# rhymes-ai/Aria

Measured on NVIDIA H100. Metric: Aria-25.3B bf16 prefill tokens/sec, higher is better.
Workload: dtype bf16

## Files before the change

aria_b200/csrc/common.cuh:

```cuda
#pragma once
#include <cuda.h>
#include <cuda_runtime.h>
#include <stdint.h>
#include <stdio.h>

#include "../../include/aria_b200.h"

namespace aria {

#define ARIA_CHECK_ARG(cond)                                                             \
  do {                                                                                   \
    if (!(cond)) {                                                                       \
      fprintf(stderr, "aria_b200: bad argument: %s (%s:%d)\n", #cond, __FILE__, __LINE__); \
      return ARIA_ERR_BAD_ARG;                                                           \
    }                                                                                    \
  } while (0)

inline int check_launch(const char* what) {
  cudaError_t e = cudaGetLastError();
  if (e != cudaSuccess) {
    fprintf(stderr, "aria_b200: launch of %s failed: %s\n", what, cudaGetErrorString(e));
    return ARIA_ERR_CUDA;
  }
  return ARIA_OK;
// ... 48 lines not shown
                   CU_TENSOR_MAP_INTERLEAVE_NONE, swizzle, CU_TENSOR_MAP_L2_PROMOTION_L2_256B,
                   CU_TENSOR_MAP_FLOAT_OOB_FILL_NONE);
  if (r == CUDA_ERROR_INVALID_CONTEXT || r == CUDA_ERROR_NOT_INITIALIZED) {
    cudaFree(0);
    r = enc(tm, dtype, rank, const_cast<void*>(ptr), gdim, gstr, bx, es,
            CU_TENSOR_MAP_INTERLEAVE_NONE, swizzle, CU_TENSOR_MAP_L2_PROMOTION_L2_256B,
            CU_TENSOR_MAP_FLOAT_OOB_FILL_NONE);
  }
  if (r != CUDA_SUCCESS) {
    fprintf(stderr, "aria_b200: cuTensorMapEncodeTiled failed (%d): rank %d ptr %p dims %llu,%llu stride %llu box %u,%u\n",
            (int)r, rank, ptr, (unsigned long long)dims[0], (unsigned long long)(rank > 1 ? dims[1] : 0),
            (unsigned long long)(rank > 1 ? strides_bytes[0] : 0), box[0], rank > 1 ? box[1] : 0);
    return ARIA_ERR_CUDA;
  }
  return ARIA_OK;
}

inline int make_tmap_2d(CUtensorMap* tm, const void* ptr, uint64_t inner, uint64_t outer, uint64_t row_stride_bytes,
                        uint32_t box_inner, uint32_t box_outer, CUtensorMapSwizzle swizzle = CU_TENSOR_MAP_SWIZZLE_128B,
                        CUtensorMapDataType dtype = CU_TENSOR_MAP_DATA_TYPE_BFLOAT16) {
  uint64_t dims[2] = {inner, outer};
  uint64_t str[1] = {row_stride_bytes};
  uint32_t box[2] = {box_inner, box_outer};
  return make_tmap_bf16_swz(tm, ptr, 2, dims, str, box, swizzle, dtype);
}

constexpr int kMaxDevices = 64;
inline int current_device() {
  int dev = 0;
  cudaGetDevice(&dev);
  return (dev >= 0 && dev < kMaxDevices) ? dev : 0;
}
inline int sm_count() {
  static int n[kMaxDevices] = {};
  const int dev = current_device();
  if (!n[dev]) {
    int v = 0;
    cudaDeviceGetAttribute(&v, cudaDevAttrMultiProcessorCount, dev);
    n[dev] = v > 0 ? v : 132;
  }
  return n[dev];
}
template <typename Kernel>
inline cudaError_t ensure_dynamic_smem(bool* flags, Kernel kern, int bytes) {
  const int dev = current_device();
  if (flags[dev]) return cudaSuccess;
  cudaError_t e = cudaFuncSetAttribute(kern, cudaFuncAttributeMaxDynamicSharedMemorySize, bytes);
  if (e == cudaSuccess) flags[dev] = true;
  else fprintf(stderr, "aria_b200: cudaFuncSetAttribute(smem=%d) failed: %s\n", bytes, cudaGetErrorString(e));
  return e;
}

template <auto kernel, typename... Args>
inline int launch_persistent(const char* name, int threads, int smem, int64_t max_tiles, cudaStream_t stream,
                             const Args&... args) {
  static bool attr_set[kMaxDevices] = {};
  if (ensure_dynamic_smem(attr_set, kernel, smem) != cudaSuccess) return ARIA_ERR_CUDA;
  int grid = sm_count();
  if (max_tiles < grid) grid = static_cast<int>(max_tiles);
  if (grid < 1) grid = 1;
  kernel<<<grid, threads, smem, stream>>>(args...);
  return check_launch(name);
}

int grouped_gemm(const void* a, const void* b, const float* b_scale, void* out, const int32_t* offsets, int64_t rows,
                 int64_t k, int64_t n, int32_t groups, int32_t epilogue, cudaStream_t stream);

}
```

aria_b200/csrc/gemm.cu:

```cuda
#include <cuda_fp8.h>

#include "gemm_common.cuh"

namespace aria {

constexpr int GEMM_STAGES = 4;
constexpr int FP8_LAND_STAGES = 3;
constexpr int FP8_CONVERT_WARPS = 3;
template <int BN, bool B_FP8 = false>
constexpr int gemm_smem_bytes() {
  return 1024  + GEMM_STAGES * (A_STAGE_BYTES + BN * BK * 2) + BM * acc_ld(BN) * 4 + 256  +
         (B_FP8 ? FP8_LAND_STAGES * BN * BK : 0);
}
static_assert(gemm_smem_bytes<128, true>() <= 232448, "fp8 landing ring must fit the opt-in shared memory of a block");

ARIA_DEVICE void e4m3x16_to_bf16(const uint4 v, uint4& lo, uint4& hi) {
  const uint32_t w[4] = {v.x, v.y, v.z, v.w};
  uint32_t o[8];
#pragma unroll
  for (int i = 0; i < 4; ++i) {
#pragma unroll
    for (int h = 0; h < 2; ++h) {
      const __half2_raw hr = __nv_cvt_fp8x2_to_halfraw2(static_cast<__nv_fp8x2_storage_t>(w[i] >> (16 * h)), __NV_E4M3);
      const float2 f = __half22float2(__half2(hr));
      o[2 * i + h] = pack_bf16(f.x, f.y);
    }
  }
  lo = make_uint4(o[0], o[1], o[2], o[3]);
  hi = make_uint4(o[4], o[5], o[6], o[7]);
}

template <int BN, bool B_MN>
ARIA_DEVICE void wgmma_tile_k16(float (&acc)[BN / 2], uint64_t da, uint64_t db) {
  if constexpr (BN == 128) wgmma_m64n128_ss<0, B_MN ? 1 : 0>(acc, da, db, 1u);
  else wgmma_m64n144_ss<0, B_MN ? 1 : 0>(acc, da, db, 1u);
}

template <int BN, bool B_MN, int EPI, bool B_FP8 = false>
__global__ void __launch_bounds__(GEMM_THREADS, 1)
gemm_kernel(const __grid_constant__ CUtensorMap tmA, const __grid_constant__ CUtensorMap tmB0,
            const __grid_constant__ CUtensorMap tmB1, const __grid_constant__ CUtensorMap tmB2, const GemmParams p) {
  constexpr int B_STAGE_BYTES = BN * BK * 2;
  constexpr int STAGE_BYTES = A_STAGE_BYTES + B_STAGE_BYTES;
  constexpr int STAGES = GEMM_STAGES;
  constexpr int ACC_LD = acc_ld(BN);
  constexpr int OUT_BN = (EPI == ARIA_EPI_SWIGLU) ? BN / 2 : BN;
  static_assert(BN == 128 || BN == 144, "tile widths with a wgmma wrapper");
  static_assert(!B_FP8 || (B_MN && BN == 128 && EPI != ARIA_EPI_HEADS), "fp8 B: grouped [G, K, N] weights, 128-wide tiles");
  constexpr int LAND_BYTES = BN * BK;

  uint8_t* smem = smem_1024();
  float* stg = reinterpret_cast<float*>(smem + STAGES * STAGE_BYTES);
  const BarrierRing<STAGES> bar(stg + BM * ACC_LD);
  const BarrierRing<FP8_LAND_STAGES> land_bar(bar.empty + STAGES);
  uint8_t* land = reinterpret_cast<uint8_t*>(bar.full) + 256;

  const int warp = threadIdx.x >> 5;
  const int lane = threadIdx.x & 31;
  const int wg = threadIdx.x >> 7;

  if (warp == 0 && lane == 0) {
    prefetch_tmap(&tmA);
    prefetch_tmap(&tmB0);
    if (p.n_seg > 1 || EPI == ARIA_EPI_SWIGLU) prefetch_tmap(&tmB1);
    if (p.n_seg > 2) prefetch_tmap(&tmB2);
    bar.init(B_FP8 ? 1 + FP8_CONVERT_WARPS : 1, CONSUMER_WARPS);
    if constexpr (B_FP8) land_bar.init(1, FP8_CONVERT_WARPS);
    fence_mbar_init();
  }
  __syncthreads();

  const int n_out_total = p.N * (EPI == ARIA_EPI_SWIGLU ? 1 : p.n_seg);
  const int n_tiles = (n_out_total + OUT_BN - 1) / OUT_BN;
  const int k_blocks = (p.K + BK - 1) / BK;
  const uint32_t smem_base = smem_u32(smem);
  const uint32_t full0 = smem_u32(bar.full), empty0 = smem_u32(bar.empty);

  if (wg == 0) {
    setmaxnreg_dec<40>();
    if (warp == 0 && elect_one()) {
      TileSched sched;
      sched.init(p, n_tiles);
      RingPos<STAGES> rp;
      RingPos<FP8_LAND_STAGES> lp;
      for (int t = blockIdx.x;; t += gridDim.x) {
        int grp, m_idx, n_idx, row0, rows;
        if (!sched.decode(t, grp, m_idx, n_idx, row0, rows)) break;
        const int a_row = row0 + m_idx * BM;
        const int bgrp = weight_block(p, grp);
        int b_c0 = 0, b_c1 = 0;
        const CUtensorMap* tb0 = &tmB0;
        const CUtensorMap* tb1 = &tmB1;
        if constexpr (B_MN) {
          b_c0 = bgrp * p.K;
        } else if constexpr (EPI == ARIA_EPI_SWIGLU) {
          b_c0 = b_c1 = n_idx * OUT_BN;
        } else {
          const int col = n_idx * BN;
          const int seg = col / p.N;
          tb0 = seg == 0 ? &tmB0 : (seg == 1 ? &tmB1 : &tmB2);
          b_c0 = col - seg * p.N + bgrp * p.b_group_rows;
        }
        for (int kb = 0; kb < k_blocks; ++kb) {
          const uint32_t fb = full0 + rp.stage * 8;
          const uint32_t sa = smem_base + rp.stage * STAGE_BYTES;
          const uint32_t sb = sa + A_STAGE_BYTES;
          mbar_wait_addr(empty0 + rp.stage * 8, rp.phase ^ 1);
          mbar_arrive_expect_tx_addr(fb, B_FP8 ? A_STAGE_BYTES : STAGE_BYTES);
          tma_load_2d_addr(sa, &tmA, fb, kb * BK, a_row);
          if constexpr (B_MN) {
            uint32_t dst = sb, box_bytes = 64 * BK * 2, bar_addr = fb;
            if constexpr (B_FP8) {
              bar_addr = smem_u32(land_bar.full) + lp.stage * 8;
              mbar_wait_addr(smem_u32(land_bar.empty) + lp.stage * 8, lp.phase ^ 1);
              mbar_arrive_expect_tx_addr(bar_addr, LAND_BYTES);
              dst = smem_u32(land) + lp.stage * LAND_BYTES;
              box_bytes = 64 * BK;
            }
            const int krow = b_c0 + kb * BK;
#pragma unroll
            for (int c = 0; c < BN / 64; ++c)
              tma_load_2d_addr(dst + c * box_bytes, &tmB0, bar_addr, tile_b_col<BN, EPI>(c * 64, n_idx, p.N), krow);
            if constexpr (B_FP8) lp.next();
          } else if constexpr (EPI == ARIA_EPI_SWIGLU) {
            tma_load_2d_addr(sb, tb0, fb, kb * BK, b_c0);
            tma_load_2d_addr(sb + (BN / 2) * BK * 2, tb1, fb, kb * BK, b_c1);
          } else {
            tma_load_2d_addr(sb, tb0, fb, kb * BK, b_c0);
          }
          rp.next();
        }
      }
    } else if constexpr (B_FP8) {
      if (warp > 0) {
        const int ct = threadIdx.x - 32;
        TileSched sched;
        sched.init(p, n_tiles);
        RingPos<STAGES> rp;
        RingPos<FP8_LAND_STAGES> lp;
        for (int t = blockIdx.x;; t += gridDim.x) {
          int grp, m_idx, n_idx, row0, rows;
          if (!sched.decode(t, grp, m_idx, n_idx, row0, rows)) break;
          for (int kb = 0; kb < k_blocks; ++kb) {
            mbar_wait_addr(smem_u32(land_bar.full) + lp.stage * 8, lp.phase);
            const uint8_t* src = land + lp.stage * LAND_BYTES;
            uint8_t* dst = smem + rp.stage * STAGE_BYTES + A_STAGE_BYTES;
#pragma unroll 1
            for (int i = ct; i < LAND_BYTES / 16; i += FP8_CONVERT_WARPS * 32) {
              const uint4 v = *reinterpret_cast<const uint4*>(src + i * 16);
              uint4 lo, hi;
              e4m3x16_to_bf16(v, lo, hi);
              const int r = (i >> 2) & 63, j = 2 * (i & 3);
              uint8_t* row = dst + (i >> 8) * (64 * BK * 2) + r * 128;
              *reinterpret_cast<uint4*>(row + ((j ^ (r & 7)) << 4)) = lo;
              *reinterpret_cast<uint4*>(row + (((j + 1) ^ (r & 7)) << 4)) = hi;
            }
            fence_proxy_async_smem();
            __syncwarp();
            if (lane == 0) {
              mbar_arrive(&bar.full[rp.stage]);
              mbar_arrive(&land_bar.empty[lp.stage]);
            }
            rp.next();
            lp.next();
          }
        }
      }
    }
  } else {
    setmaxnreg_inc<232>();
    const int cw = wg - 1;
    constexpr uint32_t b_lbo = B_MN ? 64 * BK * 2 : 16;
    constexpr uint32_t b_sbo = 1024;
    constexpr uint32_t b_kadv = (B_MN ? 16 * 128 : 32) >> 4;
    const uint64_t da0 = make_smem_desc(smem_base + cw * 64 * 128, 16, 1024);
    const uint64_t db0 = make_smem_desc(smem_base + A_STAGE_BYTES, b_lbo, b_sbo);
    const ConsumerThread ct = consumer_thread(cw, lane);
    TileSched sched;
    sched.init(p, n_tiles);
    RingPos<STAGES> rp;
    for (int t = blockIdx.x;; t += gridDim.x) {
      int grp, m_idx, n_idx, row0, rows;
      if (!sched.decode(t, grp, m_idx, n_idx, row0, rows)) break;
      float acc[BN / 2];
#pragma unroll
      for (int i = 0; i < BN / 2; ++i) acc[i] = 0.f;
      float2 bsc[BN / 8];
      if constexpr (B_FP8) load_col_scales<BN, EPI>(p, grp, n_idx, ct.frag_col, bsc);
      int prev = -1;
      for (int kb = 0; kb < k_blocks; ++kb) {
        mbar_wait_addr(full0 + rp.stage * 8, rp.phase);
        const uint64_t da = da0 + rp.stage * (STAGE_BYTES >> 4);
        const uint64_t db = db0 + rp.stage * (STAGE_BYTES >> 4);
        wgmma_fence();
#pragma unroll
        for (int k = 0; k < BK / 16; ++k) wgmma_tile_k16<BN, B_MN>(acc, da + k * 2, db + k * b_kadv);
        wgmma_commit();
        wgmma_wait<1>();
        if (prev >= 0 && lane == 0) mbar_arrive(&bar.empty[prev]);
        prev = static_cast<int>(rp.stage);
        rp.next();
      }
      wgmma_wait<0>();
      fence_regs(acc);
      if (prev >= 0 && lane == 0) mbar_arrive(&bar.empty[prev]);
      stage_and_epilogue<BN, EPI, B_FP8 ? AccScale::COL : AccScale::NONE>(p, stg, ct, acc, bsc, 1.f, 1.f, n_out_total, grp,
                                                                           m_idx, n_idx, row0, rows);
    }
  }
}

constexpr int W8_BK = 128;
static_assert(BM * W8_BK == A_STAGE_BYTES, "W8A8 A stage = bf16 A stage");

template <int EPI>
__global__ void __launch_bounds__(GEMM_THREADS, 1)
gemm_w8a8_kernel(const __grid_constant__ CUtensorMap tmA, const __grid_constant__ CUtensorMap tmB, const GemmParams p,
                 const float* __restrict__ a_scale) {
  constexpr int BN = 128;
  constexpr int STAGE_BYTES = A_STAGE_BYTES + BN * W8_BK;
  constexpr int STAGES = GEMM_STAGES;
  constexpr int ACC_LD = acc_ld(BN);
  constexpr int OUT_BN = (EPI == ARIA_EPI_SWIGLU) ? BN / 2 : BN;
  static_assert(EPI == ARIA_EPI_LINEAR || EPI == ARIA_EPI_SWIGLU, "W8A8: expert GEMM epilogues");

  uint8_t* smem = smem_1024();
  float* stg = reinterpret_cast<float*>(smem + STAGES * STAGE_BYTES);
  const BarrierRing<STAGES> bar(stg + BM * ACC_LD);

  const int warp = threadIdx.x >> 5;
  const int lane = threadIdx.x & 31;
  const int wg = threadIdx.x >> 7;

  if (warp == 0 && lane == 0) {
    prefetch_tmap(&tmA);
    prefetch_tmap(&tmB);
    bar.init(1, CONSUMER_WARPS);
    fence_mbar_init();
  }
  __syncthreads();

  const int n_tiles = (p.N + OUT_BN - 1) / OUT_BN;
  const int k_blocks = p.K / W8_BK;
  const uint32_t smem_base = smem_u32(smem);
  const uint32_t full0 = smem_u32(bar.full), empty0 = smem_u32(bar.empty);

  if (wg == 0) {
    setmaxnreg_dec<40>();
    if (warp == 0 && elect_one()) {
      TileSched sched;
      sched.init(p, n_tiles);
      RingPos<STAGES> rp;
      for (int t = blockIdx.x;; t += gridDim.x) {
        int grp, m_idx, n_idx, row0, rows;
        if (!sched.decode(t, grp, m_idx, n_idx, row0, rows)) break;
        const int a_row = row0 + m_idx * BM;
        int b_r0, b_r1;
        if constexpr (EPI == ARIA_EPI_SWIGLU) {
          b_r0 = weight_block(p, grp) * 2 * p.N + n_idx * OUT_BN;
          b_r1 = b_r0 + p.N;
        } else {
          b_r0 = weight_block(p, grp) * p.N + n_idx * BN;
// ... 68 lines not shown
  p.out_group_base = static_cast<const uint64_t*>(d->out_group_base);
  p.out_group_row0 = d->out_group_row0;
  p.group_mod = d->group_mod;
  p.b_group_rows = d->b_layout == ARIA_B_GNK ? static_cast<int>(d->n) : 0;
  p.n_seg = swiglu ? 1 : d->n_seg;
  p.act = d->act;
  for (int i = 0; i < 3; ++i) {
    p.bias[i] = static_cast<const __nv_bfloat16*>(d->bias[i]);
    p.out[i] = static_cast<__nv_bfloat16*>(d->out[i]);
  }
  p.residual = static_cast<const __nv_bfloat16*>(d->residual);
  p.ldr = d->ldr;
  p.ldo = d->ldo;
  p.head_dim = d->head_dim;
  p.head_ld = d->head_ld;
  p.rows_per_batch = d->rows_per_batch > 0 ? d->rows_per_batch : static_cast<int>(d->m);
  p.pos0 = d->pos0;
  p.stride_b = d->stride_b;
  p.stride_h = d->stride_h;
  p.rope_mask = d->rope_mask;
  p.rope_cos = static_cast<const __nv_bfloat16*>(d->rope_cos);
  p.rope_sin = static_cast<const __nv_bfloat16*>(d->rope_sin);
  p.position_ids = d->position_ids;
  p.b_scale = b_scale;
  return p;
}

static aria_gemm_desc_t grouped_desc(const void* a, const void* b, void* out, const int32_t* offsets, int64_t rows, int64_t k,
                                     int64_t n, int32_t groups, int32_t epilogue) {
  aria_gemm_desc_t d{};
  d.a = a;
  d.lda = k;
  d.m = rows;
  d.n = n;
  d.k = k;
  d.b[0] = b;
  d.n_seg = 1;
  d.b_layout = ARIA_B_GKN;
  d.num_groups = groups;
  d.group_offsets = offsets;
  d.epilogue = epilogue;
  d.out[0] = out;
  d.ldo = n;
  return d;
}

static int64_t max_tiles(const aria_gemm_desc_t* d, int BN, int64_t groups) {
  const bool swiglu = d->epilogue == ARIA_EPI_SWIGLU;
  const int out_bn = swiglu ? BN / 2 : BN;
  const int64_t n_out_total = d->n * (swiglu ? 1 : d->n_seg);
  return (n_out_total + out_bn - 1) / out_bn * ((d->m + BM - 1) / BM + groups);
}

static int gemm_run(const aria_gemm_desc_t* d, const float* b_scale, cudaStream_t stream) {
  ARIA_CHECK_ARG(d != nullptr);
  ARIA_CHECK_ARG(d->a && d->b[0] && d->out[0]);
  ARIA_CHECK_ARG(d->m >= 0 && d->n > 0 && d->k > 0);
  ARIA_CHECK_ARG(d->n % 8 == 0 && d->k % 8 == 0 && d->lda % 8 == 0);
  ARIA_CHECK_ARG(d->n_seg >= 1 && d->n_seg <= 3);
  ARIA_CHECK_ARG(d->num_groups >= 1 && (d->group_mod >= 0 || d->num_groups % (-d->group_mod) == 0));
  ARIA_CHECK_ARG((reinterpret_cast<uintptr_t>(d->a) & 15) == 0 && (reinterpret_cast<uintptr_t>(d->out[0]) & 15) == 0);
  if (d->m == 0) return ARIA_OK;
  const bool b_mn = d->b_layout == ARIA_B_GKN;
  const bool b_gnk = d->b_layout == ARIA_B_GNK;
  const bool swiglu = d->epilogue == ARIA_EPI_SWIGLU;
  if (b_mn) {
    ARIA_CHECK_ARG(d->n_seg == 1);
    ARIA_CHECK_ARG(d->k % BK == 0 || (d->num_groups == 1 && d->group_mod == 0));
    ARIA_CHECK_ARG(d->n % 64 == 0);
    ARIA_CHECK_ARG(d->epilogue != ARIA_EPI_HEADS);
  } else {
    ARIA_CHECK_ARG(d->num_groups == 1 || d->n_seg == 1);
    if (swiglu) ARIA_CHECK_ARG(d->n_seg == 2 && d->b[1]);
    if (b_gnk) ARIA_CHECK_ARG(d->n_seg == 1 && !swiglu && d->epilogue == ARIA_EPI_LINEAR && d->n % 128 == 0);
    else ARIA_CHECK_ARG(d->num_groups == 1);
  }
  if (d->num_groups > 1) ARIA_CHECK_ARG(d->group_offsets != nullptr);
  if (d->group_counts) ARIA_CHECK_ARG(d->group_offsets != nullptr);
  if (d->out_group_base) ARIA_CHECK_ARG(d->out_group_row0 != nullptr && d->epilogue == ARIA_EPI_LINEAR && d->group_offsets != nullptr);
  ARIA_CHECK_ARG(d->a_rows == 0 || d->a_rows >= d->m);

  int BN = 128;
  if (d->epilogue == ARIA_EPI_HEADS) {
    ARIA_CHECK_ARG(d->head_dim > 0 && d->head_dim % 8 == 0 && d->head_ld >= d->head_dim && d->n % d->head_dim == 0);
    if (d->rope_mask) ARIA_CHECK_ARG(d->head_dim == 128 && d->rope_cos && d->rope_sin);
    if (d->n % 128 != 0) {
      ARIA_CHECK_ARG(!d->rope_mask && d->n % 144 == 0);
      BN = 144;
    }
    for (int s = 0; s < d->n_seg; ++s) ARIA_CHECK_ARG(d->out[s] && d->b[s]);
  } else {
    if (swiglu) ARIA_CHECK_ARG(d->n % 64 == 0);
    if (d->n_seg > 1 && !swiglu) ARIA_CHECK_ARG(d->n % BN == 0);
  }

  CUtensorMap tmA, tmB[3];
  int rc = make_tmap_2d(&tmA, d->a, d->k, d->a_rows > 0 ? d->a_rows : d->m, d->lda * 2, BK, BM);
  if (rc) return rc;
  if (b_mn) {
    const uint64_t ncols = swiglu ? 2 * d->n : d->n;
    const uint64_t n_weights = d->group_mod > 0 ? d->group_mod : (d->group_mod < 0 ? d->num_groups / (-d->group_mod) : d->num_groups);
    rc = b_scale ? make_tmap_2d(&tmB[0], d->b[0], ncols, n_weights * d->k, ncols, 64, BK, CU_TENSOR_MAP_SWIZZLE_NONE,
                                CU_TENSOR_MAP_DATA_TYPE_UINT8)
                 : make_tmap_2d(&tmB[0], d->b[0], ncols, n_weights * d->k, ncols * 2, 64, BK);
    if (rc) return rc;
    tmB[1] = tmB[0];
    tmB[2] = tmB[0];
  } else {
    const int nb = swiglu ? 2 : d->n_seg;
    const uint32_t box_rows = swiglu ? BN / 2 : BN;
    for (int s = 0; s < 3; ++s) {
      const void* ptr = s < nb ? d->b[s] : d->b[0];
      const uint64_t b_rows = b_gnk ? static_cast<uint64_t>(d->group_mod > 0 ? d->group_mod : (d->group_mod < 0 ? d->num_groups / (-d->group_mod) : d->num_groups)) * d->n : d->n;
      rc = make_tmap_2d(&tmB[s], ptr, d->k, b_rows, d->k * 2, BK, box_rows);
      if (rc) return rc;
    }
  }

  const GemmParams p = gemm_params(d, b_scale);
  const int64_t tiles = max_tiles(d, BN, d->num_groups > 1 ? d->num_groups : 0);
#define ARIA_LAUNCH(BN_, MN_, EPI_, ...)                                                                                     \
  return launch_persistent<gemm_kernel<BN_, MN_, EPI_, ##__VA_ARGS__>>("gemm_kernel", GEMM_THREADS,                          \
                                                                       gemm_smem_bytes<BN_, ##__VA_ARGS__>(), tiles, stream, \
                                                                       tmA, tmB[0], tmB[1], tmB[2], p)
  if (b_scale) {
    if (swiglu) ARIA_LAUNCH(128, true, ARIA_EPI_SWIGLU, true);
    ARIA_LAUNCH(128, true, ARIA_EPI_LINEAR, true);
  }
  if (d->epilogue == ARIA_EPI_HEADS) {
    if (BN == 128) ARIA_LAUNCH(128, false, ARIA_EPI_HEADS);
    ARIA_LAUNCH(144, false, ARIA_EPI_HEADS);
  }
  if (swiglu) {
    if (b_mn) ARIA_LAUNCH(128, true, ARIA_EPI_SWIGLU);
    ARIA_LAUNCH(128, false, ARIA_EPI_SWIGLU);
  }
  if (b_mn) ARIA_LAUNCH(128, true, ARIA_EPI_LINEAR);
  ARIA_LAUNCH(128, false, ARIA_EPI_LINEAR);
#undef ARIA_LAUNCH
}

extern "C" int aria_gemm(const aria_gemm_desc_t* d, aria_stream_t stream) {
  return gemm_run(d, nullptr, reinterpret_cast<cudaStream_t>(stream));
}

int aria::grouped_gemm(const void* a, const void* b, const float* b_scale, void* out, const int32_t* offsets, int64_t rows,
                       int64_t k, int64_t n, int32_t groups, int32_t epilogue, cudaStream_t stream) {
  const aria_gemm_desc_t d = grouped_desc(a, b, out, offsets, rows, k, n, groups, epilogue);
  return gemm_run(&d, b_scale, stream);
}

extern "C" int aria_grouped_gemm(const void* a, const void* b, void* out, const int32_t* group_offsets, int64_t rows,
                                 int64_t k, int64_t n, int32_t num_groups, aria_stream_t stream) {
  return grouped_gemm(a, b, nullptr, out, group_offsets, rows, k, n, num_groups, ARIA_EPI_LINEAR,
                      reinterpret_cast<cudaStream_t>(stream));
}

extern "C" int aria_grouped_gemm_fp8(const void* a, const void* b_fp8, const float* b_scale, void* out,
                                     const int32_t* group_offsets, int64_t rows, int64_t k, int64_t n, int32_t num_groups,
                                     int32_t epilogue, aria_stream_t stream) {
  ARIA_CHECK_ARG(a && b_fp8 && b_scale && out && group_offsets);
  ARIA_CHECK_ARG(rows >= 0 && k > 0 && n > 0 && k % BK == 0 && n % 64 == 0 && num_groups >= 1);
  ARIA_CHECK_ARG(epilogue == ARIA_EPI_LINEAR || epilogue == ARIA_EPI_SWIGLU);
  ARIA_CHECK_ARG((reinterpret_cast<uintptr_t>(a) & 15) == 0 && (reinterpret_cast<uintptr_t>(b_fp8) & 15) == 0 &&
                 (reinterpret_cast<uintptr_t>(b_scale) & 15) == 0 && (reinterpret_cast<uintptr_t>(out) & 15) == 0);
  return grouped_gemm(a, b_fp8, b_scale, out, group_offsets, rows, k, n, num_groups, epilogue,
                      reinterpret_cast<cudaStream_t>(stream));
}

extern "C" int aria_grouped_gemm_w8a8(const void* a_fp8, const float* a_scale, const void* b_fp8_nk, const float* b_scale,
                                      void* out, const int32_t* group_offsets, int64_t rows, int64_t k, int64_t n,
                                      int32_t num_groups, int32_t epilogue, aria_stream_t stream_) {
  ARIA_CHECK_ARG(a_fp8 && a_scale && b_fp8_nk && b_scale && out && group_offsets);
  ARIA_CHECK_ARG(rows >= 0 && rows < (int64_t(1) << 31) && k > 0 && n > 0 && k % W8_BK == 0 && n % 64 == 0 && num_groups >= 1);
  ARIA_CHECK_ARG(k <= (1 << 30) && n <= (1 << 29) && static_cast<int64_t>(num_groups) * n * 2 < (int64_t(1) << 31));
  ARIA_CHECK_ARG(epilogue == ARIA_EPI_LINEAR || epilogue == ARIA_EPI_SWIGLU);
  ARIA_CHECK_ARG((reinterpret_cast<uintptr_t>(a_fp8) & 15) == 0 && (reinterpret_cast<uintptr_t>(b_fp8_nk) & 15) == 0 &&
                 (reinterpret_cast<uintptr_t>(b_scale) & 15) == 0 && (reinterpret_cast<uintptr_t>(out) & 15) == 0 &&
                 (reinterpret_cast<uintptr_t>(a_scale) & 3) == 0);
  if (rows == 0) return ARIA_OK;
  const bool swiglu = epilogue == ARIA_EPI_SWIGLU;
  const aria_gemm_desc_t d = grouped_desc(a_fp8, b_fp8_nk, out, group_offsets, rows, k, n, num_groups, epilogue);
  const GemmParams p = gemm_params(&d, b_scale);

  CUtensorMap tmA, tmB;
  int rc = make_tmap_2d(&tmA, a_fp8, k, rows, k, W8_BK, BM, CU_TENSOR_MAP_SWIZZLE_128B, CU_TENSOR_MAP_DATA_TYPE_UINT8);
  if (rc) return rc;
  rc = make_tmap_2d(&tmB, b_fp8_nk, k, num_groups * (swiglu ? 2 * n : n), k, W8_BK, 64, CU_TENSOR_MAP_SWIZZLE_128B,
                    CU_TENSOR_MAP_DATA_TYPE_UINT8);
  if (rc) return rc;

  const int64_t tiles = max_tiles(&d, 128, num_groups);
  constexpr int SMEM = gemm_smem_bytes<128>();
  cudaStream_t stream = reinterpret_cast<cudaStream_t>(stream_);
  if (swiglu)
    return launch_persistent<gemm_w8a8_kernel<ARIA_EPI_SWIGLU>>("gemm_w8a8_kernel", GEMM_THREADS, SMEM, tiles, stream, tmA,
                                                                 tmB, p, a_scale);
  return launch_persistent<gemm_w8a8_kernel<ARIA_EPI_LINEAR>>("gemm_w8a8_kernel", GEMM_THREADS, SMEM, tiles, stream, tmA, tmB,
                                                              p, a_scale);
}

extern "C" int aria_abi_version(void) { return 3; }
extern "C" const char* aria_build_arch(void) { return "sm_90a"; }
```

aria_b200/csrc/gemm_common.cuh:

```cuda
#pragma once
#include "common.cuh"
#include "ptx.cuh"

namespace aria {

constexpr int BM = 128;
constexpr int BK = 64;
constexpr int A_STAGE_BYTES = BM * BK * 2;
constexpr int GEMM_THREADS = 384;
constexpr int CONSUMER_WARPS = 8;
constexpr int acc_ld(int BN) { return BN + 4; }

struct GemmParams {
  int M, N, K;
  int num_groups;
  const int32_t* group_offsets;
  const int32_t* group_counts;
  const uint64_t* out_group_base;
  const int32_t* out_group_row0;
  int b_group_rows;
  int group_mod;
  int n_seg;
  int act;
  const __nv_bfloat16* bias[3];
  const __nv_bfloat16* residual;
  int64_t ldr;
  __nv_bfloat16* out[3];
  int64_t ldo;
  int head_dim, head_ld, rows_per_batch, pos0;
  int64_t stride_b, stride_h;
  int rope_mask;
  const __nv_bfloat16* rope_cos;
  const __nv_bfloat16* rope_sin;
  const int32_t* position_ids;
  const float* b_scale;
};

ARIA_DEVICE int weight_block(const GemmParams& p, int grp) {
  return p.group_mod > 0 ? grp % p.group_mod : (p.group_mod < 0 ? grp / (-p.group_mod) : grp);
}

ARIA_DEVICE uint8_t* smem_1024() {
  extern __shared__ uint8_t smem_raw[];
  return reinterpret_cast<uint8_t*>((reinterpret_cast<uintptr_t>(smem_raw) + 1023) & ~uintptr_t(1023));
}

template <int STAGES>
struct BarrierRing {
  uint64_t* full;
  uint64_t* empty;
  ARIA_DEVICE explicit BarrierRing(void* at) : full(static_cast<uint64_t*>(at)), empty(full + STAGES) {}
  ARIA_DEVICE void init(uint32_t full_arrivals, uint32_t empty_arrivals) const {
    for (int i = 0; i < STAGES; ++i) {
      mbar_init(&full[i], full_arrivals);
      mbar_init(&empty[i], empty_arrivals);
    }
  }
};

template <int STAGES>
struct RingPos {
  uint32_t stage = 0, phase = 0;
  ARIA_DEVICE void next() {
    const bool wrap = ++stage == STAGES;
    stage = wrap ? 0 : stage;
    phase ^= wrap;
  }
};

template <int BN, int EPI>
ARIA_DEVICE int tile_b_col(int x, int n_idx, int N) {
  constexpr int OUT_BN = BN / 2;
  if constexpr (EPI == ARIA_EPI_SWIGLU) return x < OUT_BN ? n_idx * OUT_BN + x : N + n_idx * OUT_BN + x - OUT_BN;
  else return n_idx * BN + x;
}

struct ConsumerThread {
  int cw, frag_row, frag_col, epi_row, half;
};
ARIA_DEVICE ConsumerThread consumer_thread(int cw, int lane) {
  const int tid = threadIdx.x & 127;
  return {cw, cw * 64 + (tid >> 5) * 16 + (lane >> 2), 2 * (lane & 3), cw * 64 + (tid & 63), tid >> 6};
}

template <int BN, int EPI>
ARIA_DEVICE void load_col_scales(const GemmParams& p, int grp, int n_idx, int frag_col, float2 (&bsc)[BN / 8]) {
  const int ncols = EPI == ARIA_EPI_SWIGLU ? 2 * p.N : p.N;
  const float* srow = p.b_scale + static_cast<int64_t>(weight_block(p, grp)) * ncols;
// ... 328 lines not shown
```

aria_b200/csrc/gemm_wgrad.cu:

```cuda
#include "gemm_common.cuh"

namespace aria {

struct WgradParams {
  int Md, Nd, G;
  int n_src;
  const int32_t* offs;
  __nv_bfloat16* out;
};

constexpr int WG_BN = 128;
constexpr int WG_STAGES = 6;
constexpr int WG_STAGE_BYTES = 64 * BM * 2 + 64 * WG_BN * 2;

__global__ void __launch_bounds__(GEMM_THREADS, 1)
wgrad_kernel(const __grid_constant__ CUtensorMap tmA, const __grid_constant__ CUtensorMap tmB, const WgradParams p) {
  uint8_t* smem = smem_1024();
  const BarrierRing<WG_STAGES> bar(smem + WG_STAGES * WG_STAGE_BYTES);
  const int warp = threadIdx.x >> 5, lane = threadIdx.x & 31, wg = threadIdx.x >> 7;

  if (warp == 0 && lane == 0) {
    prefetch_tmap(&tmA);
    prefetch_tmap(&tmB);
    bar.init(1, CONSUMER_WARPS);
// ... 73 lines not shown
            else named_bar_sync(2, 128);
          }
          wgmma_fence();
          for (int k = 0; k < kmax; ++k) wgmma_m64n128_ss<1, 1>(acc, da + k * (2048 >> 4), db + k * (2048 >> 4), 1u);
          wgmma_commit();
          wgmma_wait<1>();
          if (prev >= 0 && lane == 0) mbar_arrive(&bar.empty[prev]);
          prev = static_cast<int>(rp.stage);
          rp.next();
        }
      }
      wgmma_wait<0>();
      fence_regs(acc);
      if (prev >= 0 && lane == 0) mbar_arrive(&bar.empty[prev]);
#pragma unroll
      for (int h = 0; h < 2; ++h) {
        const int m = mi * BM + ct.frag_row + 8 * h;
        if (m >= p.Md) continue;
        __nv_bfloat16* orow = p.out + (static_cast<int64_t>(g) * p.Md + m) * p.Nd + ni * WG_BN;
#pragma unroll
        for (int j = 0; j < WG_BN / 8; ++j) {
          if (ni * WG_BN + 8 * j + 8 <= p.Nd)
            *reinterpret_cast<uint32_t*>(orow + 8 * j + ct.frag_col) = pack_bf16(acc[4 * j + 2 * h], acc[4 * j + 2 * h + 1]);
        }
      }
    }
  }
}

}

using namespace aria;

extern "C" int aria_grouped_wgrad(const void* a, int64_t lda, const void* b, int64_t ldb, void* out, const int32_t* group_offsets,
                                  int64_t rows, int64_t md, int64_t nd, int32_t num_groups, int32_t num_sources,
                                  aria_stream_t stream_) {
  cudaStream_t stream = reinterpret_cast<cudaStream_t>(stream_);
  ARIA_CHECK_ARG(a && b && out && group_offsets && rows >= 0 && md > 0 && nd > 0 && num_groups >= 1 && num_sources >= 1);
  ARIA_CHECK_ARG(md % 8 == 0 && nd % 8 == 0 && lda % 8 == 0 && ldb % 8 == 0 && lda >= md && ldb >= nd);
  CUtensorMap tmA, tmB;
  int rc = make_tmap_2d(&tmA, a, md, rows > 0 ? rows : 1, lda * 2, 64, 64);
  if (rc) return rc;
  rc = make_tmap_2d(&tmB, b, nd, rows > 0 ? rows : 1, ldb * 2, 64, 64);
  if (rc) return rc;
  WgradParams p{};
  p.Md = static_cast<int>(md);
  p.Nd = static_cast<int>(nd);
  p.G = num_groups;
  p.n_src = num_sources;
  p.offs = group_offsets;
  p.out = static_cast<__nv_bfloat16*>(out);
  constexpr int SMEM = WG_STAGES * WG_STAGE_BYTES + 1024 + 256;
  const int64_t tiles = static_cast<int64_t>(num_groups) * ((md + BM - 1) / BM) * ((nd + WG_BN - 1) / WG_BN);
  return launch_persistent<wgrad_kernel>("wgrad_kernel", GEMM_THREADS, SMEM, tiles, stream, tmA, tmB, p);
}
```

aria_b200/csrc/ptx.cuh:

```cuda
#pragma once
#include <cuda.h>
#include <cuda_bf16.h>
#include <cuda_runtime.h>
#include <stdint.h>

namespace aria {

#define ARIA_DEVICE __device__ __forceinline__

ARIA_DEVICE uint32_t smem_u32(const void* p) { return static_cast<uint32_t>(__cvta_generic_to_shared(p)); }

ARIA_DEVICE uint32_t elect_one() {
  uint32_t pred = 0;
  asm volatile(
      "{\n\t.reg .pred P;\n\t"
      "elect.sync _|P, 0xffffffff;\n\t"
      "selp.b32 %0, 1, 0, P;\n\t}\n"
      : "=r"(pred));
  return pred;
}

ARIA_DEVICE void mbar_init(uint64_t* bar, uint32_t count) {
  asm volatile("mbarrier.init.shared::cta.b64 [%0], %1;" ::"r"(smem_u32(bar)), "r"(count));
}
ARIA_DEVICE void fence_mbar_init() { asm volatile("fence.mbarrier_init.release.cluster;" ::: "memory"); }
ARIA_DEVICE void fence_proxy_async_smem() { asm volatile("fence.proxy.async.shared::cta;" ::: "memory"); }

ARIA_DEVICE void mbar_arrive_expect_tx(uint64_t* bar, uint32_t bytes) {
  asm volatile("mbarrier.arrive.expect_tx.shared::cta.b64 _, [%0], %1;" ::"r"(smem_u32(bar)), "r"(bytes)
               : "memory");
}
ARIA_DEVICE void mbar_arrive(uint64_t* bar) {
  asm volatile("mbarrier.arrive.shared::cta.b64 _, [%0];" ::"r"(smem_u32(bar)) : "memory");
}
ARIA_DEVICE bool mbar_try_wait(uint64_t* bar, uint32_t parity) {
  uint32_t ok;
  asm volatile(
      "{\n\t.reg .pred P;\n\t"
      "mbarrier.try_wait.parity.shared::cta.b64 P, [%1], %2;\n\t"
      "selp.b32 %0, 1, 0, P;\n\t}\n"
      : "=r"(ok) : "r"(smem_u32(bar)), "r"(parity) : "memory");
  return ok != 0;
}
ARIA_DEVICE void mbar_wait_addr(uint32_t addr, uint32_t parity) {
  uint32_t ok = 0;
  long long t0 = 0;
  for (uint32_t spin = 0;; ++spin) {
    asm volatile(
        "{\n\t.reg .pred P;\n\t"
        "mbarrier.try_wait.parity.shared::cta.b64 P, [%1], %2;\n\t"
        "selp.b32 %0, 1, 0, P;\n\t}\n"
        : "=r"(ok) : "r"(addr), "r"(parity) : "memory");
    if (ok) return;
    if ((spin & 0xFFF) == 0xFFF) {
      const long long now = clock64();
      if (t0 == 0) t0 = now;
      if (now - t0 > 4000000000ll) __trap();
    }
  }
}
ARIA_DEVICE void mbar_wait(uint64_t* bar, uint32_t parity) { mbar_wait_addr(smem_u32(bar), parity); }
ARIA_DEVICE void mbar_arrive_expect_tx_addr(uint32_t bar_addr, uint32_t bytes) {
  asm volatile("mbarrier.arrive.expect_tx.shared::cta.b64 _, [%0], %1;" ::"r"(bar_addr), "r"(bytes) : "memory");
}

ARIA_DEVICE void tma_load_2d_addr(uint32_t dst, const CUtensorMap* m, uint32_t bar_addr, int c0, int c1) {
  asm volatile(
      "cp.async.bulk.tensor.2d.shared::cluster.global.mbarrier::complete_tx::bytes [%0], [%1, {%3, %4}], [%2];"
      ::"r"(dst), "l"(reinterpret_cast<uint64_t>(m)), "r"(bar_addr), "r"(c0), "r"(c1)
      : "memory");
}
ARIA_DEVICE void prefetch_tmap(const CUtensorMap* m) {
  asm volatile("prefetch.tensormap [%0];" ::"l"(reinterpret_cast<uint64_t>(m)) : "memory");
}
ARIA_DEVICE void tma_load_2d(void* dst, const CUtensorMap* m, uint64_t* bar, int c0, int c1) {
  asm volatile(
      "cp.async.bulk.tensor.2d.shared::cluster.global.mbarrier::complete_tx::bytes [%0], [%1, {%3, %4}], [%2];"
      ::"r"(smem_u32(dst)), "l"(reinterpret_cast<uint64_t>(m)), "r"(smem_u32(bar)), "r"(c0), "r"(c1)
      : "memory");
}
ARIA_DEVICE void tma_load_3d(void* dst, const CUtensorMap* m, uint64_t* bar, int c0, int c1, int c2) {
  asm volatile(
      "cp.async.bulk.tensor.3d.shared::cluster.global.mbarrier::complete_tx::bytes [%0], [%1, {%3, %4, %5}], [%2];"
      ::"r"(smem_u32(dst)), "l"(reinterpret_cast<uint64_t>(m)), "r"(smem_u32(bar)), "r"(c0), "r"(c1), "r"(c2)
      : "memory");
}
ARIA_DEVICE void tma_load_4d(void* dst, const CUtensorMap* m, uint64_t* bar, int c0, int c1, int c2, int c3) {
  asm volatile(
      "cp.async.bulk.tensor.4d.shared::cluster.global.mbarrier::complete_tx::bytes [%0], [%1, {%3, %4, %5, %6}], [%2];"
      ::"r"(smem_u32(dst)), "l"(reinterpret_cast<uint64_t>(m)), "r"(smem_u32(bar)), "r"(c0), "r"(c1), "r"(c2),
      "r"(c3)
      : "memory");
}

ARIA_DEVICE uint64_t make_smem_desc(uint32_t smem_addr, uint32_t lbo_bytes, uint32_t sbo_bytes) {
  uint64_t d = 0;
  d |= static_cast<uint64_t>((smem_addr & 0x3FFFF) >> 4);
  d |= static_cast<uint64_t>((lbo_bytes >> 4) & 0x3FFF) << 16;
  d |= static_cast<uint64_t>((sbo_bytes >> 4) & 0x3FFF) << 32;
  d |= 1ull << 62;
  return d;
}
ARIA_DEVICE uint64_t make_smem_desc_sw32(uint32_t smem_addr, uint32_t sbo_bytes) {
  uint64_t d = 0;
  d |= static_cast<uint64_t>((smem_addr & 0x3FFFF) >> 4);
  d |= static_cast<uint64_t>(1) << 16;
  d |= static_cast<uint64_t>((sbo_bytes >> 4) & 0x3FFF) << 32;
  d |= 3ull << 62;
  return d;
}
ARIA_DEVICE void wgmma_fence() { asm volatile("wgmma.fence.sync.aligned;" ::: "memory"); }
ARIA_DEVICE void wgmma_commit() { asm volatile("wgmma.commit_group.sync.aligned;" ::: "memory"); }
template <int N> ARIA_DEVICE void wgmma_wait() { asm volatile("wgmma.wait_group.sync.aligned %0;" ::"n"(N) : "memory"); }
template <int R> ARIA_DEVICE void fence_regs(float (&d)[R]) {
#pragma unroll
  for (int i = 0; i < R; ++i) asm volatile("" : "+f"(d[i])::"memory");
}
ARIA_DEVICE void named_bar_sync(uint32_t id, uint32_t threads) { asm volatile("bar.sync %0, %1;" ::"r"(id), "r"(threads) : "memory"); }
ARIA_DEVICE void named_bar_arrive(uint32_t id, uint32_t threads) { asm volatile("bar.arrive %0, %1;" ::"r"(id), "r"(threads) : "memory"); }

template <int TA, int TB>
ARIA_DEVICE void wgmma_m64n128_ss(float (&d)[64], uint64_t da, uint64_t db, uint32_t scale_d) {
// ... 89 lines not shown
```

Measured before the change: 16630.

## Pair CTAs in 2-CTA clusters that multicast shared B tiles for dense GEMMs

Dense bf16 GEMMs with long K and at least two M tiles now launch as 2-CTA clusters. The two CTAs take adjacent M tiles of the same N tile, and each loads half of the B tile and multicasts it to both. Empty-slot releases are sent to both CTAs' barriers so a stage is reused only after both consumers finish. This halves B traffic from global/L2 per pair, at the cost of cluster scheduling limits, cross-CTA lockstep and an extra clamp for odd M-tile counts.

```diff
diff --git a/aria_b200/csrc/common.cuh b/aria_b200/csrc/common.cuh
--- a/aria_b200/csrc/common.cuh
+++ b/aria_b200/csrc/common.cuh
@@ -124,14 +124,49 @@
 }
 
 template <auto kernel, typename... Args>
-inline int launch_persistent(const char* name, int threads, int smem, int64_t max_tiles, cudaStream_t stream,
+inline int launch_persistent(const char* name, int threads, int smem, int64_t max_tiles, int cluster, cudaStream_t stream,
                              const Args&... args) {
   static bool attr_set[kMaxDevices] = {};
+  static int max_clusters[kMaxDevices] = {};
   if (ensure_dynamic_smem(attr_set, kernel, smem) != cudaSuccess) return ARIA_ERR_CUDA;
-  int grid = sm_count();
-  if (max_tiles < grid) grid = static_cast<int>(max_tiles);
-  if (grid < 1) grid = 1;
-  kernel<<<grid, threads, smem, stream>>>(args...);
+  if (cluster <= 1) {
+    int grid = sm_count();
+    if (max_tiles < grid) grid = static_cast<int>(max_tiles);
+    if (grid < 1) grid = 1;
+    kernel<<<grid, threads, smem, stream>>>(args...);
+    return check_launch(name);
+  }
+  cudaLaunchConfig_t cfg{};
+  cudaLaunchAttribute attr{};
+  attr.id = cudaLaunchAttributeClusterDimension;
+  attr.val.clusterDim.x = cluster;
+  attr.val.clusterDim.y = 1;
+  attr.val.clusterDim.z = 1;
+  cfg.blockDim = dim3(threads);
+  cfg.dynamicSmemBytes = smem;
+  cfg.stream = stream;
+  cfg.attrs = &attr;
+  cfg.numAttrs = 1;
+  const int dev = current_device();
+  if (!max_clusters[dev]) {
+    cfg.gridDim = dim3(sm_count() / cluster * cluster);
+    int n = 0;
+    const cudaError_t e = cudaOccupancyMaxActiveClusters(&n, kernel, &cfg);
+    if (e != cudaSuccess || n < 1) {
+      fprintf(stderr, "aria_b200: no cluster of %d x %s fits (%s)\n", cluster, name, cudaGetErrorString(e));
+      return ARIA_ERR_CUDA;
+    }
+    max_clusters[dev] = n;
+  }
+  int64_t clusters = max_clusters[dev];
+  if (max_tiles < clusters) clusters = max_tiles;
+  if (clusters < 1) clusters = 1;
+  cfg.gridDim = dim3(static_cast<unsigned>(clusters * cluster));
+  const cudaError_t e = cudaLaunchKernelEx(&cfg, kernel, args...);
+  if (e != cudaSuccess) {
+    fprintf(stderr, "aria_b200: launch of %s failed: %s\n", name, cudaGetErrorString(e));
+    return ARIA_ERR_CUDA;
+  }
   return check_launch(name);
 }
 
diff --git a/aria_b200/csrc/gemm.cu b/aria_b200/csrc/gemm.cu
--- a/aria_b200/csrc/gemm.cu
+++ b/aria_b200/csrc/gemm.cu
@@ -58,35 +58,41 @@
   const int warp = threadIdx.x >> 5;
   const int lane = threadIdx.x & 31;
   const int wg = threadIdx.x >> 7;
+  const bool pair = !B_MN && p.cta_pair;
+  const int n_cta = pair ? 2 : 1;
+  const int rank = pair ? static_cast<int>(cluster_ctarank()) : 0;
 
   if (warp == 0 && lane == 0) {
     prefetch_tmap(&tmA);
     prefetch_tmap(&tmB0);
     if (p.n_seg > 1 || EPI == ARIA_EPI_SWIGLU) prefetch_tmap(&tmB1);
     if (p.n_seg > 2) prefetch_tmap(&tmB2);
-    bar.init(B_FP8 ? 1 + FP8_CONVERT_WARPS : 1, CONSUMER_WARPS);
+    bar.init(B_FP8 ? 1 + FP8_CONVERT_WARPS : 1, CONSUMER_WARPS * n_cta);
     if constexpr (B_FP8) land_bar.init(1, FP8_CONVERT_WARPS);
     fence_mbar_init();
   }
-  __syncthreads();
+  if (pair) cluster_sync();
+  else __syncthreads();
 
   const int n_out_total = p.N * (EPI == ARIA_EPI_SWIGLU ? 1 : p.n_seg);
   const int n_tiles = (n_out_total + OUT_BN - 1) / OUT_BN;
   const int k_blocks = (p.K + BK - 1) / BK;
   const uint32_t smem_base = smem_u32(smem);
   const uint32_t full0 = smem_u32(bar.full), empty0 = smem_u32(bar.empty);
+  const int t0 = blockIdx.x / n_cta, t_step = gridDim.x / n_cta;
 
   if (wg == 0) {
     setmaxnreg_dec<40>();
     if (warp == 0 && elect_one()) {
       TileSched sched;
-      sched.init(p, n_tiles);
+      sched.init(p, n_tiles, BM * n_cta);
       RingPos<STAGES> rp;
       RingPos<FP8_LAND_STAGES> lp;
-      for (int t = blockIdx.x;; t += gridDim.x) {
+      for (int t = t0;; t += t_step) {
         int grp, m_idx, n_idx, row0, rows;
         if (!sched.decode(t, grp, m_idx, n_idx, row0, rows)) break;
-        const int a_row = row0 + m_idx * BM;
+        m_idx = m_idx * n_cta + rank;
+        const int a_row = row0 + min(m_idx, (rows - 1) / BM) * BM;
         const int bgrp = weight_block(p, grp);
         int b_c0 = 0, b_c1 = 0;
         const CUtensorMap* tb0 = &tmB0;
@@ -122,11 +128,17 @@
             for (int c = 0; c < BN / 64; ++c)
               tma_load_2d_addr(dst + c * box_bytes, &tmB0, bar_addr, tile_b_col<BN, EPI>(c * 64, n_idx, p.N), krow);
             if constexpr (B_FP8) lp.next();
-          } else if constexpr (EPI == ARIA_EPI_SWIGLU) {
-            tma_load_2d_addr(sb, tb0, fb, kb * BK, b_c0);
-            tma_load_2d_addr(sb + (BN / 2) * BK * 2, tb1, fb, kb * BK, b_c1);
           } else {
-            tma_load_2d_addr(sb, tb0, fb, kb * BK, b_c0);
+#pragma unroll
+            for (int h = 0; h < 2; ++h) {
+              if (pair && h != rank) continue;
+              const uint32_t dst = sb + h * (BN / 2) * BK * 2;
+              const CUtensorMap* tb = EPI == ARIA_EPI_SWIGLU && h ? tb1 : tb0;
+              int b_row = EPI == ARIA_EPI_SWIGLU ? (h ? b_c1 : b_c0) : b_c0 + h * (BN / 2);
+              if (b_row - bgrp * p.b_group_rows >= p.N) b_row = b_c0;
+              if (pair) tma_load_2d_multicast_addr(dst, tb, fb, kb * BK, b_row, 0x3);
+              else tma_load_2d_addr(dst, tb, fb, kb * BK, b_row);
+            }
           }
           rp.next();
         }
@@ -176,12 +188,21 @@
     const uint64_t da0 = make_smem_desc(smem_base + cw * 64 * 128, 16, 1024);
     const uint64_t db0 = make_smem_desc(smem_base + A_STAGE_BYTES, b_lbo, b_sbo);
     const ConsumerThread ct = consumer_thread(cw, lane);
+    auto release = [&](int stage) {
+      if (pair) {
+        mbar_arrive_cluster(empty0 + stage * 8, 0);
+        mbar_arrive_cluster(empty0 + stage * 8, 1);
+      } else {
+        mbar_arrive(&bar.empty[stage]);
+      }
+    };
     TileSched sched;
-    sched.init(p, n_tiles);
+    sched.init(p, n_tiles, BM * n_cta);
     RingPos<STAGES> rp;
-    for (int t = blockIdx.x;; t += gridDim.x) {
+    for (int t = t0;; t += t_step) {
       int grp, m_idx, n_idx, row0, rows;
       if (!sched.decode(t, grp, m_idx, n_idx, row0, rows)) break;
+      m_idx = m_idx * n_cta + rank;
       float acc[BN / 2];
 #pragma unroll
       for (int i = 0; i < BN / 2; ++i) acc[i] = 0.f;
@@ -197,17 +218,18 @@
         for (int k = 0; k < BK / 16; ++k) wgmma_tile_k16<BN, B_MN>(acc, da + k * 2, db + k * b_kadv);
         wgmma_commit();
         wgmma_wait<1>();
-        if (prev >= 0 && lane == 0) mbar_arrive(&bar.empty[prev]);
+        if (prev >= 0 && lane == 0) release(prev);
         prev = static_cast<int>(rp.stage);
         rp.next();
       }
       wgmma_wait<0>();
       fence_regs(acc);
-      if (prev >= 0 && lane == 0) mbar_arrive(&bar.empty[prev]);
+      if (prev >= 0 && lane == 0) release(prev);
       stage_and_epilogue<BN, EPI, B_FP8 ? AccScale::COL : AccScale::NONE>(p, stg, ct, acc, bsc, 1.f, 1.f, n_out_total, grp,
                                                                            m_idx, n_idx, row0, rows);
     }
   }
+  if (pair) cluster_sync();
 }
 
 constexpr int W8_BK = 128;
@@ -382,6 +404,8 @@
   return (n_out_total + out_bn - 1) / out_bn * ((d->m + BM - 1) / BM + groups);
 }
 
+constexpr int PAIR_MIN_K_BLOCKS = 64;
+
 static int gemm_run(const aria_gemm_desc_t* d, const float* b_scale, cudaStream_t stream) {
   ARIA_CHECK_ARG(d != nullptr);
   ARIA_CHECK_ARG(d->a && d->b[0] && d->out[0]);
@@ -438,7 +462,7 @@
     tmB[2] = tmB[0];
   } else {
     const int nb = swiglu ? 2 : d->n_seg;
-    const uint32_t box_rows = swiglu ? BN / 2 : BN;
+    const uint32_t box_rows = BN / 2;
     for (int s = 0; s < 3; ++s) {
       const void* ptr = s < nb ? d->b[s] : d->b[0];
       const uint64_t b_rows = b_gnk ? static_cast<uint64_t>(d->group_mod > 0 ? d->group_mod : (d->group_mod < 0 ? d->num_groups / (-d->group_mod) : d->num_groups)) * d->n : d->n;
@@ -447,12 +471,16 @@
     }
   }
 
-  const GemmParams p = gemm_params(d, b_scale);
-  const int64_t tiles = max_tiles(d, BN, d->num_groups > 1 ? d->num_groups : 0);
-#define ARIA_LAUNCH(BN_, MN_, EPI_, ...)                                                                                     \
-  return launch_persistent<gemm_kernel<BN_, MN_, EPI_, ##__VA_ARGS__>>("gemm_kernel", GEMM_THREADS,                          \
-                                                                       gemm_smem_bytes<BN_, ##__VA_ARGS__>(), tiles, stream, \
-                                                                       tmA, tmB[0], tmB[1], tmB[2], p)
+  GemmParams p = gemm_params(d, b_scale);
+  const int64_t m_tiles = (d->m + BM - 1) / BM;
+  p.cta_pair = !b_mn && d->num_groups == 1 && !d->group_offsets && m_tiles >= 2 && d->k >= PAIR_MIN_K_BLOCKS * BK;
+  const int64_t tiles = p.cta_pair ? max_tiles(d, BN, 0) / m_tiles * ((m_tiles + 1) / 2)
+                                   : max_tiles(d, BN, d->num_groups > 1 ? d->num_groups : 0);
+  const int cluster = p.cta_pair ? 2 : 1;
+#define ARIA_LAUNCH(BN_, MN_, EPI_, ...)                                                                           \
+  return launch_persistent<gemm_kernel<BN_, MN_, EPI_, ##__VA_ARGS__>>("gemm_kernel", GEMM_THREADS,                \
+                                                                       gemm_smem_bytes<BN_, ##__VA_ARGS__>(), tiles, \
+                                                                       cluster, stream, tmA, tmB[0], tmB[1], tmB[2], p)
   if (b_scale) {
     if (swiglu) ARIA_LAUNCH(128, true, ARIA_EPI_SWIGLU, true);
     ARIA_LAUNCH(128, true, ARIA_EPI_LINEAR, true);
@@ -524,9 +552,9 @@
   constexpr int SMEM = gemm_smem_bytes<128>();
   cudaStream_t stream = reinterpret_cast<cudaStream_t>(stream_);
   if (swiglu)
-    return launch_persistent<gemm_w8a8_kernel<ARIA_EPI_SWIGLU>>("gemm_w8a8_kernel", GEMM_THREADS, SMEM, tiles, stream, tmA,
+    return launch_persistent<gemm_w8a8_kernel<ARIA_EPI_SWIGLU>>("gemm_w8a8_kernel", GEMM_THREADS, SMEM, tiles, 1, stream, tmA,
                                                                  tmB, p, a_scale);
-  return launch_persistent<gemm_w8a8_kernel<ARIA_EPI_LINEAR>>("gemm_w8a8_kernel", GEMM_THREADS, SMEM, tiles, stream, tmA, tmB,
+  return launch_persistent<gemm_w8a8_kernel<ARIA_EPI_LINEAR>>("gemm_w8a8_kernel", GEMM_THREADS, SMEM, tiles, 1, stream, tmA, tmB,
                                                               p, a_scale);
 }
 
diff --git a/aria_b200/csrc/gemm_common.cuh b/aria_b200/csrc/gemm_common.cuh
--- a/aria_b200/csrc/gemm_common.cuh
+++ b/aria_b200/csrc/gemm_common.cuh
@@ -34,6 +34,7 @@
   const __nv_bfloat16* rope_sin;
   const int32_t* position_ids;
   const float* b_scale;
+  int cta_pair;
 };
 
 ARIA_DEVICE int weight_block(const GemmParams& p, int grp) {
diff --git a/aria_b200/csrc/gemm_wgrad.cu b/aria_b200/csrc/gemm_wgrad.cu
--- a/aria_b200/csrc/gemm_wgrad.cu
+++ b/aria_b200/csrc/gemm_wgrad.cu
@@ -149,5 +149,5 @@
   p.out = static_cast<__nv_bfloat16*>(out);
   constexpr int SMEM = WG_STAGES * WG_STAGE_BYTES + 1024 + 256;
   const int64_t tiles = static_cast<int64_t>(num_groups) * ((md + BM - 1) / BM) * ((nd + WG_BN - 1) / WG_BN);
-  return launch_persistent<wgrad_kernel>("wgrad_kernel", GEMM_THREADS, SMEM, tiles, stream, tmA, tmB, p);
+  return launch_persistent<wgrad_kernel>("wgrad_kernel", GEMM_THREADS, SMEM, tiles, 1, stream, tmA, tmB, p);
 }
diff --git a/aria_b200/csrc/ptx.cuh b/aria_b200/csrc/ptx.cuh
--- a/aria_b200/csrc/ptx.cuh
+++ b/aria_b200/csrc/ptx.cuh
@@ -63,11 +63,35 @@
 ARIA_DEVICE void mbar_arrive_expect_tx_addr(uint32_t bar_addr, uint32_t bytes) {
   asm volatile("mbarrier.arrive.expect_tx.shared::cta.b64 _, [%0], %1;" ::"r"(bar_addr), "r"(bytes) : "memory");
 }
+ARIA_DEVICE void mbar_arrive_cluster(uint32_t bar_addr, uint32_t cta) {
+  asm volatile(
+      "{\n\t.reg .b32 remote;\n\t"
+      "mapa.shared::cluster.u32 remote, %0, %1;\n\t"
+      "mbarrier.arrive.shared::cluster.b64 _, [remote];\n\t}\n"
+      ::"r"(bar_addr), "r"(cta) : "memory");
+}
+
+ARIA_DEVICE uint32_t cluster_ctarank() {
+  uint32_t r;
+  asm volatile("mov.u32 %0, %%cluster_ctarank;" : "=r"(r));
+  return r;
+}
+ARIA_DEVICE void cluster_sync() {
+  asm volatile("barrier.cluster.arrive.release;\n\tbarrier.cluster.wait.acquire;" ::: "memory");
+}
 
 ARIA_DEVICE void tma_load_2d_addr(uint32_t dst, const CUtensorMap* m, uint32_t bar_addr, int c0, int c1) {
   asm volatile(
       "cp.async.bulk.tensor.2d.shared::cluster.global.mbarrier::complete_tx::bytes [%0], [%1, {%3, %4}], [%2];"
       ::"r"(dst), "l"(reinterpret_cast<uint64_t>(m)), "r"(bar_addr), "r"(c0), "r"(c1)
+      : "memory");
+}
+ARIA_DEVICE void tma_load_2d_multicast_addr(uint32_t dst, const CUtensorMap* m, uint32_t bar_addr, int c0, int c1,
+                                            uint16_t cta_mask) {
+  asm volatile(
+      "cp.async.bulk.tensor.2d.shared::cluster.global.mbarrier::complete_tx::bytes.multicast::cluster"
+      " [%0], [%1, {%3, %4}], [%2], %5;"
+      ::"r"(dst), "l"(reinterpret_cast<uint64_t>(m)), "r"(bar_addr), "r"(c0), "r"(c1), "h"(cta_mask)
       : "memory");
 }
 ARIA_DEVICE void prefetch_tmap(const CUtensorMap* m) {
```

Result: no change. 16690 (median of 6 runs) (+0.4%).
